# adithom/KWS

Measured on AMD Instinct MI355X. Metric: utterances/sec fwd+bwd, T=99 feat=32 hidden=128, bs=4096 at 1/2/4/8 GPUs, higher is better.
Workload: dtype f32 (split-precision MFMA: exact 3xbf16 planes, fp16 two-plane forward state product; fp32 accumulate)

## Files before the change

include/fastgrnn_hip.h:

```cpp
#ifndef FASTGRNN_HIP_H
#define FASTGRNN_HIP_H

#include <stddef.h>
#include <stdint.h>

#ifdef __cplusplus
extern "C" {
#endif

#define FASTGRNN_HIP_ABI_VERSION 1

typedef enum fastgrnn_status {
  FASTGRNN_OK = 0,
  FASTGRNN_ERR_NULL_POINTER = 1,
  FASTGRNN_ERR_BAD_SHAPE = 2,
  FASTGRNN_ERR_BAD_NONLINEARITY = 3,
  FASTGRNN_ERR_BAD_DTYPE = 4,
  FASTGRNN_ERR_WORKSPACE = 5,
  FASTGRNN_ERR_LAUNCH = 6,
  FASTGRNN_ERR_UNSUPPORTED = 7
} fastgrnn_status;

typedef enum fastgrnn_dtype {
  FASTGRNN_F32 = 0,
  FASTGRNN_F64 = 1,
  FASTGRNN_BF16_IO = 2
} fastgrnn_dtype;

typedef enum fastgrnn_nonlinearity {
  FASTGRNN_NL_SIGMOID = 0, FASTGRNN_NL_RELU = 1, FASTGRNN_NL_TANH = 2,
  FASTGRNN_NL_QUANT_TANH = 3, FASTGRNN_NL_QUANT_SIGM = 4, FASTGRNN_NL_QUANT_SIGM4 = 5
} fastgrnn_nonlinearity;

#define FASTGRNN_FLAG_FORCE_GENERIC 1u
#define FASTGRNN_FLAG_FORCE_F32_MFMA 2u
#define FASTGRNN_FLAG_SAVE_PREACT 4u
#define FASTGRNN_FLAG_FWD_4WAVE 8u
#define FASTGRNN_FLAG_BATCH_MAJOR 16u
#define FASTGRNN_FLAG_X_BFT 128u
#define FASTGRNN_FLAG_FWD_BF16X3 64u
#define FASTGRNN_FLAG_GRAD_LAST 256u
#define FASTGRNN_FLAG_HS_LAST 512u
#define FASTGRNN_FLAG_PREACT_AFFINE 1024u
#define FASTGRNN_FLAG_BN_TRAIN 2048u
#define FASTGRNN_FLAG_ZERO_EXTEND 4096u
#define FASTGRNN_FLAG_NO_INPUT_GRAD 8192u

typedef struct fastgrnn_desc {
  int32_t T, B, F, H;
  int32_t w_rank, u_rank;
  int32_t gate_nl;
  int32_t update_nl;
  int32_t dtype;
  uint32_t flags;
} fastgrnn_desc;

typedef struct fastgrnn_params {
  const void *w, *u;
  const void *w1, *w2, *u1, *u2;
  const void *bias_gate;
  const void *bias_update;
  const void *zeta, *nu;
} fastgrnn_params;

typedef struct fastgrnn_grads {
  void *d_x;
  void *d_bias_gate;
  void *d_bias_update;
  void *d_zeta;
  void *d_nu;
  void *d_h0;
  void *d_w, *d_u;
  void *d_w1, *d_w2;
  void *d_u1, *d_u2;
} fastgrnn_grads;

int fastgrnn_hip_abi_version(void);
const char *fastgrnn_hip_status_string(int status);

int fastgrnn_hip_kernel_path(const fastgrnn_desc *d, int direction);

typedef struct fastgrnn_zext_plan {
  int32_t forward, backward;
  int32_t Hp, Fp;
  int32_t dx_optional, reserved;
  size_t saved_bytes;
} fastgrnn_zext_plan;
int fastgrnn_hip_zero_extend_plan(const fastgrnn_desc *d, fastgrnn_zext_plan *out);

typedef struct fastgrnn_plan {
  int32_t path[2];
  int32_t forward_ws_optional, dx_optional;
  int32_t rank_space_cols, reserved;
  size_t workspace_bytes[2];
  fastgrnn_zext_plan zext;
} fastgrnn_plan;
int fastgrnn_hip_plan(const fastgrnn_desc *d, fastgrnn_plan *out);

size_t fastgrnn_hip_forward_workspace_bytes(const fastgrnn_desc *d);
size_t fastgrnn_hip_backward_workspace_bytes(const fastgrnn_desc *d);

int fastgrnn_hip_forward_unroll(const fastgrnn_desc *d, const fastgrnn_params *p,
                                const void *x, const void *h0,
                                void *hs, void *z_s, void *c_s,
                                void *workspace, size_t workspace_bytes, void *stream);

int fastgrnn_hip_forward_unroll_affine(const fastgrnn_desc *d, const fastgrnn_params *p,
                                       const void *gate_scale, const void *update_scale,
                                       const void *x, const void *h0, void *hs,
                                       void *workspace, size_t workspace_bytes, void *stream);

int fastgrnn_hip_backward_unroll(const fastgrnn_desc *d, const fastgrnn_params *p,
                                 const void *grad_hs, const void *x, const void *hs,
                                 const void *z_s, const void *c_s, const void *h0,
                                 const fastgrnn_grads *g,
                                 void *workspace, size_t workspace_bytes, void *stream);

int fastgrnn_hip_forward(const fastgrnn_desc *d, const fastgrnn_params *p,
                         const void *x, const void *old_h,
                         void *new_h, void *z, void *c,
                         void *workspace, size_t workspace_bytes, void *stream);

int fastgrnn_hip_backward(const fastgrnn_desc *d, const fastgrnn_params *p,
                          const void *grad_h, const void *x, const void *old_h,
                          const void *z, const void *c,
                          const fastgrnn_grads *g,
                          void *workspace, size_t workspace_bytes, void *stream);

size_t fastgrnn_hip_head_workspace_bytes(int32_t B, int32_t H, int32_t C);
// ... 44 lines not shown
```

kws_amd/_lib.py:

```python
from __future__ import annotations

import ctypes as C
import os

_HERE = os.path.dirname(os.path.abspath(__file__))
LIB_PATH = os.environ.get("FASTGRNN_HIP_LIB") or os.path.join(_HERE, "csrc", "libfastgrnn_hip.so")

ABI_VERSION = 1

F32, F64, BF16_IO = 0, 1, 2
FLAG_FORCE_GENERIC = 1
FLAG_FORCE_F32_MFMA = 2
FLAG_SAVE_PREACT = 4
FLAG_FWD_4WAVE = 8
FLAG_FWD_BF16X3 = 64
FLAG_X_BFT = 128
FLAG_GRAD_LAST = 256
FLAG_HS_LAST = 512
FLAG_BATCH_MAJOR = 16
FLAG_PREACT_AFFINE = 1024
FLAG_BN_TRAIN = 2048
FLAG_ZERO_EXTEND = 4096
FLAG_NO_INPUT_GRAD = 8192

NONLINEARITY = {"sigmoid": 0, "relu": 1, "tanh": 2, "quantTanh": 3, "quantSigm": 4, "quantSigm4": 5}

EXPORTS = (
    "fastgrnn_hip_abi_version", "fastgrnn_hip_status_string", "fastgrnn_hip_kernel_path",
    "fastgrnn_hip_forward_workspace_bytes", "fastgrnn_hip_backward_workspace_bytes",
    "fastgrnn_hip_forward_unroll", "fastgrnn_hip_backward_unroll",
    "fastgrnn_hip_forward", "fastgrnn_hip_backward",
    "fastgrnn_hip_head_workspace_bytes", "fastgrnn_hip_head_xent", "fastgrnn_hip_debug_poison_cu_state",
    "fastgrnn_hip_frame_gemm", "fastgrnn_hip_forward_unroll_affine",
    "fastgrnn_hip_bn_train_supported", "fastgrnn_hip_bn_train_forward_workspace_bytes",
    "fastgrnn_hip_bn_train_backward_workspace_bytes", "fastgrnn_hip_bn_train_forward", "fastgrnn_hip_bn_train_backward",
    "fastgrnn_hip_zero_extend_plan", "fastgrnn_hip_plan",
)


class Desc(C.Structure):
    _fields_ = [("T", C.c_int32), ("B", C.c_int32), ("F", C.c_int32), ("H", C.c_int32),
                ("w_rank", C.c_int32), ("u_rank", C.c_int32),
                ("gate_nl", C.c_int32), ("update_nl", C.c_int32),
                ("dtype", C.c_int32), ("flags", C.c_uint32)]


class Params(C.Structure):
    _fields_ = [(n, C.c_void_p) for n in
                ("w", "u", "w1", "w2", "u1", "u2", "bias_gate", "bias_update", "zeta", "nu")]


class Grads(C.Structure):
    _fields_ = [(n, C.c_void_p) for n in
                ("d_x", "d_bias_gate", "d_bias_update", "d_zeta", "d_nu", "d_h0",
                 "d_w", "d_u", "d_w1", "d_w2", "d_u1", "d_u2")]


class BnLayer(C.Structure):
    _fields_ = [("gamma", C.c_void_p), ("beta", C.c_void_p), ("running_mean", C.c_void_p),
                ("running_var", C.c_void_p), ("num_batches_tracked", C.c_void_p),
                ("eps", C.c_double), ("momentum", C.c_double)]


class BnParams(C.Structure):
    _fields_ = [("w", BnLayer), ("u", BnLayer), ("gate", BnLayer), ("update", BnLayer)]


class BnGrads(C.Structure):
    _fields_ = [(n, C.c_void_p) for n in
                ("d_gamma_w", "d_beta_w", "d_gamma_u", "d_beta_u", "d_gamma_gate", "d_beta_gate",
                 "d_gamma_update", "d_beta_update")]


class ZextPlan(C.Structure):
    _fields_ = [("forward", C.c_int32), ("backward", C.c_int32), ("Hp", C.c_int32), ("Fp", C.c_int32),
                ("dx_optional", C.c_int32), ("reserved", C.c_int32), ("saved_bytes", C.c_size_t)]


class Plan(C.Structure):
    _fields_ = [("path", C.c_int32 * 2), ("forward_ws_optional", C.c_int32), ("dx_optional", C.c_int32),
                ("rank_space_cols", C.c_int32), ("reserved", C.c_int32), ("workspace_bytes", C.c_size_t * 2),
                ("zext", ZextPlan)]


class FastGRNNLibraryError(RuntimeError):
    pass


_lib = None


def load():
    global _lib
    if _lib is not None:
        return _lib
    if not os.path.exists(LIB_PATH):
        raise FastGRNNLibraryError(
            "libfastgrnn_hip.so not found at %s -- build it first: "
            "python -c 'import __graft_entry__ as g; g.build()'  (or make -C kws_amd/csrc). "
            "kws_amd has no CPU or eager fallback." % LIB_PATH)
    lib = C.CDLL(LIB_PATH)
    for name in EXPORTS:
        if not hasattr(lib, name):
            raise FastGRNNLibraryError("%s does not export %s" % (LIB_PATH, name))
    vp, sz, i32 = C.c_void_p, C.c_size_t, C.c_int
    DP, PP, GP = C.POINTER(Desc), C.POINTER(Params), C.POINTER(Grads)
# ... 55 lines not shown
```

kws_amd/csrc/kernels_split.hip:

```cpp
#include "split_common.h"

namespace fastgrnn {
namespace {

template <int GATE, int AUX, bool RAGGED>
__global__ __launch_bounds__(256) ONE_WAVE_PER_SIMD void fwd_scan_split(
    int Tn, int B, int rsT, int rsB, const float* __restrict__ x, const float* __restrict__ h0,
    const float* __restrict__ w, const float* __restrict__ u,
    const float* __restrict__ bz, const float* __restrict__ bh,
    const float* __restrict__ zeta, const float* __restrict__ nu,
    float* __restrict__ hs, float* __restrict__ zs, float* __restrict__ cs) {
  constexpr int H = 128, F = 32, MT = 2, KS = H / 32;
  __shared__ u32x4 hl[2][3][KS * 4 * 16];

  const int tid = threadIdx.x;
  const int wv = __builtin_amdgcn_readfirstlane(tid >> 6);
  const int l = tid & 63, i = l & 15, g = l >> 4;
  const int b = blockIdx.x * 16 + i;
  const bool valid = !RAGGED || b < B;
  const int bc = valid ? b : B - 1;
  const int n0 = wv * 32 + g * 8;
  const int myfrag = (wv * 4 + g) * 16 + i;

  Frag3 Uf[MT][KS], Wf[MT];
// ... 68 lines not shown
#pragma unroll
      for (int r = 0; r < 4; ++r) {
        const float pre = a[r];
        const float z = gate_act<GATE>(pre + bzv[mt][r]);
        const float c = ftanh(pre + bhv[mt][r]);
        hown[mt][r] = (sz * (1.0f - z) + sn) * c + hown[mt][r] * z;
        gout.z[mt][r] = (AUX == 2) ? pre : z; gout.c[mt][r] = c;
      }
    };
    constexpr int NM = (KS + 1) * 6;
    SPLIT_STAMP(0)
    if (!FIRST) store_step(t - 1, gprev);
    const f32x4 acc0 = tile_chain(0);
    if (!FIRST) {
      constexpr int NST = (AUX == 1 ? 3 : AUX == 2 ? 2 : 1) * MT, PER = NM / (NST + 1);
#pragma unroll
      for (int j = 0; j < NST; ++j) {
        __builtin_amdgcn_sched_group_barrier(0x008, PER, 0);
        __builtin_amdgcn_sched_group_barrier(0x040, 1, 0);
      }
    }
    __builtin_amdgcn_sched_barrier(0);
    SPLIT_STAMP(1)
    const f32x4 acc1 = tile_chain(1);
    tile_epilogue(0, acc0);
#pragma unroll
    for (int k = 0; k < NM; ++k) {
      __builtin_amdgcn_sched_group_barrier(0x008, 1, 0);
      __builtin_amdgcn_sched_group_barrier(0x002, 3, 0);
    }
    __builtin_amdgcn_sched_barrier(0);
    SPLIT_STAMP(2)
    {
      float probe = acc1[0];
      keep_alive(probe, xB);
#pragma unroll
      for (int s = 0; s < KS; ++s) keep_alive(probe, hB[s]);
      completion_read(probe);
      __builtin_amdgcn_sched_barrier(0);
    }
    tile_epilogue(1, acc1);
    const Frag3 f = split3(hown[0], hown[1]);
#pragma unroll
    for (int p = 0; p < 3; ++p) hl[cur ^ 1][p][myfrag] = f.p[p];
    __builtin_amdgcn_sched_barrier(0);
    SPLIT_STAMP(3)
    lds_barrier();
    SPLIT_STAMP(4)
  };

  Feat xa, xb;
  Gates ga, gb;
  load_x(0, xa);
  __syncthreads();
  step(std::true_type{}, 0, 0, xa, xb, gb, ga);
  int t = 1;
  for (; t + 1 < Tn; t += 2) {
    step(std::false_type{}, t, 1, xb, xa, ga, gb);
    step(std::false_type{}, t + 1, 0, xa, xb, gb, ga);
  }
  if (t < Tn) {
    step(std::false_type{}, t, 1, xb, xa, ga, gb);
    store_step(Tn - 1, gb);
  } else {
    store_step(Tn - 1, ga);
  }
  {
    float probe = hown[0][0];
#pragma unroll
    for (int mt = 0; mt < MT; ++mt) {
      keep_alive(probe, Wf[mt]);
#pragma unroll
      for (int s = 0; s < KS; ++s) keep_alive(probe, Uf[mt][s]);
    }
  }
#ifdef FASTGRNN_DIAG_STAMPS
  if (blockIdx.x == 7 && l == 0) { for (int k = 0; k < 8; ++k) g_sdiag[wv][k] = dsum[k]; }
#endif
}

constexpr int W8_ROWH = 272;
constexpr int W8_ROWX = 80;

constexpr bool fwd_w8_built(int gate, int aux, bool bf, bool f16h, bool prein, bool uq, bool aff) {
  const bool ref_gate = gate <= FASTGRNN_NL_TANH;
  if (f16h && !gate_bounds_state(gate)) return false;
  if (aff) return ref_gate && !bf && !uq && (aux == 0 || aux == 3);
  if (uq) return !bf && !prein && (aux == 0 || aux == 2);
  if (bf && prein) return ref_gate && (aux == 0 || aux == 2);
  return true;
}
template <int GATE, int AUX, bool RAGGED, bool BF = false, bool F16H = true, bool PREIN = false, bool UQ = false,
          bool AFF = false>
__global__ __launch_bounds__(512) void fwd_scan_split_w8(
    int Tn, int B, int rsT, int rsB, int mode, const float* __restrict__ x, const float* __restrict__ h0,
    const float* __restrict__ w, const float* __restrict__ u,
    const float* __restrict__ bz, const float* __restrict__ bh,
    const float* __restrict__ zeta, const float* __restrict__ nu,
    float* __restrict__ hs, float* __restrict__ zs, float* __restrict__ cs,
    const float* __restrict__ sg = nullptr, const float* __restrict__ sc = nullptr) {
  constexpr int H = 128, F = 32, KS = H / 32;
  __shared__ __attribute__((aligned(16))) unsigned char hpl[2][3][16 * W8_ROWH];
  __shared__ __attribute__((aligned(16))) unsigned char xpl[PREIN ? 1 : 2][3][PREIN ? 16 : 16 * W8_ROWX];
  float* const pbuf = (AUX == 1) ? cs : zs;

  const int tid = threadIdx.x;
  const int wv = __builtin_amdgcn_readfirstlane(tid >> 6);
  const int l = tid & 63, i = l & 15, g = l >> 4;
  const int b = blockIdx.x * 16 + i;
  const bool valid = !RAGGED || b < B;
  const int bc = valid ? b : B - 1;
  const int n0 = wv * 16 + g * 4;
  const bool xbft = (mode & 1) != 0;
  constexpr bool hs_last = AUX == 3;
  const int xu = tid >> 5, xf = tid & 31;
  const int xb = blockIdx.x * 16 + xu;
  const int xbc = (!RAGGED || xb < B) ? xb : B - 1;

  const f32x4 bzv = ld4(bz + n0), bhv = ld4(bh + n0);
  const f32x4 sgv = AFF ? ld4(sg + n0) : f32x4{1.f, 1.f, 1.f, 1.f}, scv = AFF ? ld4(sc + n0) : f32x4{1.f, 1.f, 1.f, 1.f};
  f32x4 hown = ld4(h0 + (size_t)bc * H + n0);
  const float sz = fsigmoid(zeta[0]), sn = fsigmoid(nu[0]);

  bool use_h16 = false;
  if constexpr (F16H) {
    __shared__ float hmax_s[8];
    float hm = fmaxf(fmaxf(fabsf(hown[0]), fabsf(hown[1])), fmaxf(fabsf(hown[2]), fabsf(hown[3])));
    if (!(hm == hm)) hm = 3.0e38f;
#pragma unroll
    for (int m = 1; m < 64; m <<= 1) hm = fmaxf(hm, __shfl_xor(hm, m));
    if (l == 0) hmax_s[wv] = hm;
    __syncthreads();
#pragma unroll
    for (int k2 = 0; k2 < 8; ++k2) hm = fmaxf(hm, hmax_s[k2]);
    use_h16 = __builtin_amdgcn_readfirstlane((int)(hm + (float)Tn + 2.0f < 3.0e4f)) != 0;
  }

  auto scan = [&](auto h16_tag) __attribute__((always_inline)) {
  constexpr bool H16 = decltype(h16_tag)::value;
  Frag3 Uf[KS], Wf;
  Frag2h Uh[KS];
  float u_unscale = 1.0f;
  {
    const int nA = wv * 16 + i;
    f32x4 ulo[KS], uhi[KS];
    float umax = 0.f;
#pragma unroll
    for (int s2 = 0; s2 < KS; ++s2) {
      const float* up = u + (size_t)nA * H + 32 * s2 + 8 * g;
      ulo[s2] = ld4(up); uhi[s2] = ld4(up + 4);
#pragma unroll
      for (int j = 0; j < 4; ++j) umax = fmaxf(umax, fmaxf(fabsf(ulo[s2][j]), fabsf(uhi[s2][j])));
    }
    if (H16) {
#pragma unroll
      for (int m = 1; m < 64; m <<= 1) umax = fmaxf(umax, __shfl_xor(umax, m));
      int e = 0;
      if (umax > 0.f && umax < 3.0e38f) (void)frexpf(umax, &e);
      e = e < -100 ? -100 : (e > 100 ? 100 : e);
      const float u_scale = ldexpf(1.0f, 13 - e);
      u_unscale = ldexpf(1.0f, e - 13);
#pragma unroll
      for (int s2 = 0; s2 < KS; ++s2) Uh[s2] = split2h8(ulo[s2] * u_scale, uhi[s2] * u_scale);
    } else {
#pragma unroll
      for (int s2 = 0; s2 < KS; ++s2) Uf[s2] = split3(ulo[s2], uhi[s2]);
    }
    if (!PREIN) {
      const float* wp = w + (size_t)nA * F + 8 * g;
      Wf = split3(ld4(wp), ld4(wp + 4));
    }
  }

  auto publish_h = [&](int buf) __attribute__((always_inline)) {
    const unsigned off = i * W8_ROWH + n0 * 2;
    if (H16) {
      uint2 hi, lo;
      split2h(hown[0], hown[1], hi.x, lo.x); split2h(hown[2], hown[3], hi.y, lo.y);
      *reinterpret_cast<uint2*>(&hpl[buf][0][off]) = hi;
      *reinterpret_cast<uint2*>(&hpl[buf][1][off]) = lo;
      return;
    }
    uint2 q0, q1, q2;
    split_quad(hown, q0, q1, q2);
    *reinterpret_cast<uint2*>(&hpl[buf][0][off]) = q0;
    *reinterpret_cast<uint2*>(&hpl[buf][1][off]) = q1;
    *reinterpret_cast<uint2*>(&hpl[buf][2][off]) = q2;
  };
  auto publish_x = [&](int buf, float v) __attribute__((always_inline)) {
    unsigned short s0, s1, s2;
    split_one(v, s0, s1, s2);
    const unsigned off = xu * W8_ROWX + xf * 2;
    *reinterpret_cast<unsigned short*>(&xpl[buf][0][off]) = s0;
    *reinterpret_cast<unsigned short*>(&xpl[buf][1][off]) = s1;
    *reinterpret_cast<unsigned short*>(&xpl[buf][2][off]) = s2;
  };
  const size_t xbase = xbft ? ((size_t)xbc * F + xf) * Tn : (size_t)xbc * rsB * F + xf;
  const size_t xstep = xbft ? 1 : (size_t)rsT * F;
  auto load_x = [&](int t) __attribute__((always_inline)) {
    const size_t e = xbase + (size_t)t * xstep;
    return BF ? bf16_to_f32(reinterpret_cast<const unsigned short*>(x)[e]) : x[e];
  };
  auto load_p = [&](int t) __attribute__((always_inline)) {
    return ld4(pbuf + ((size_t)t * rsT + (size_t)bc * rsB) * H + n0);
  };
  auto store_step = [&](int t, const f32x4 aux) __attribute__((always_inline)) {
    if (hs_last && t != Tn - 1) return;
    if (RAGGED) lds_writes_landed();
    if (valid) {
      const size_t o = hs_last ? (size_t)b * H + n0 : ((size_t)t * rsT + (size_t)b * rsB) * H + n0;
      if (BF) st4_bf16(reinterpret_cast<unsigned short*>(hs) + o, hown); else st4(hs + o, hown);
      if (AUX == 2) st4(zs + o, aux);
    }
  };

  publish_h(0);
  float xnext = 0.f;
  f32x4 pnext = f32x4{0.f, 0.f, 0.f, 0.f};
  if (PREIN) {
    pnext = load_p(0);
  } else {
    publish_x(0, load_x(0));
    xnext = load_x(Tn > 1 ? 1 : 0);
  }
  __syncthreads();

  f32x4 aux_prev = f32x4{0.f, 0.f, 0.f, 0.f};
#ifdef FASTGRNN_DIAG_STAMPS
  unsigned long long dsum[8] = {0, 0, 0, 0, 0, 0, 0, 0}, dlast = 0;
  asm volatile("s_memtime %0\n\ts_waitcnt lgkmcnt(0)" : "=s"(dlast)::"memory");
#endif
  for (int t = 0; t < Tn; ++t) {
    const int cur = t & 1;
    SPLIT_STAMP(0)
    const float xpub = xnext;
    const f32x4 pcur = pnext;
    if (PREIN) pnext = load_p(t + 1 < Tn ? t + 1 : Tn - 1);
    else xnext = load_x(t + 2 < Tn ? t + 2 : Tn - 1);
    Frag3 xB, hB[KS];
    Frag2h hH[KS];
    if (!PREIN) {
#pragma unroll
      for (int p = 0; p < 3; ++p) xB.p[p] = *reinterpret_cast<const u32x4*>(&xpl[cur][p][i * W8_ROWX + 16 * g]);
    }
#pragma unroll
    for (int s2 = 0; s2 < KS; ++s2) {
      if (H16) {
        hH[s2].hi = *reinterpret_cast<const u32x4*>(&hpl[cur][0][i * W8_ROWH + 64 * s2 + 16 * g]);
        hH[s2].lo = *reinterpret_cast<const u32x4*>(&hpl[cur][1][i * W8_ROWH + 64 * s2 + 16 * g]);
      } else {
#pragma unroll
        for (int p = 0; p < 3; ++p)
          hB[s2].p[p] = *reinterpret_cast<const u32x4*>(&hpl[cur][p][i * W8_ROWH + 64 * s2 + 16 * g]);
      }
    }
    if (t > 0) store_step(t - 1, aux_prev);
    if (!PREIN) publish_x(cur ^ 1, xpub);
    __builtin_amdgcn_sched_barrier(0);
    SPLIT_STAMP(1)
    f32x4 a = f32x4{0.f, 0.f, 0.f, 0.f}, alo = a;
    if (PREIN) {
      a = pcur;
    } else if (BF) {
      alo = mfma_bf16(Wf.p[2], xB.p[0], alo);
      alo = mfma_bf16(Wf.p[1], xB.p[0], alo);
      a = mfma_bf16(Wf.p[0], xB.p[0], a);
    } else {
      mfma6_hl(Wf, xB, a, alo);
    }
    if (H16) {
      f32x4 ah = f32x4{0.f, 0.f, 0.f, 0.f}, ahlo = ah;
#pragma unroll
      for (int s2 = 0; s2 < KS; ++s2) mfma3h_hl(Uh[s2], hH[s2], ah, ahlo);
      a = (a + alo) + (ah + ahlo) * u_unscale;
    } else {
#pragma unroll
      for (int s2 = 0; s2 < KS; ++s2) mfma6_hl(Uf[s2], hB[s2], a, alo);
      a += alo;
    }
    f32x4 zq, cq;
    SPLIT_STAMP(2)
#pragma unroll
    for (int r = 0; r < 4; ++r) {
      const float z = gate_act<GATE>(AFF ? fmaf(a[r], sgv[r], bzv[r]) : a[r] + bzv[r]);
      const float c = UQ ? fminf(fmaxf(a[r] + bhv[r], -1.0f), 1.0f)
                         : ftanh(AFF ? fmaf(a[r], scv[r], bhv[r]) : a[r] + bhv[r]);
      hown[r] = (sz * (1.0f - z) + sn) * c + hown[r] * z;
      zq[r] = z; cq[r] = c;
    }
    if (AUX == 1 && RAGGED) lds_writes_landed();
    if (AUX == 1 && valid) {
      const size_t o = ((size_t)t * rsT + (size_t)b * rsB) * H + n0;
      st4(zs + o, zq); st4(cs + o, cq);
    }
    aux_prev = a;
    publish_h(cur ^ 1);
    SPLIT_STAMP(3)
    lds_barrier();
    SPLIT_STAMP(4)
  }
#ifdef FASTGRNN_DIAG_STAMPS
  if (blockIdx.x == 7 && l == 0) { for (int k2 = 0; k2 < 8; ++k2) g_sdiag[wv][k2] = dsum[k2]; }
#endif
  store_step(Tn - 1, aux_prev);
  };
  if constexpr (F16H) {
    if (use_h16) scan(std::true_type{}); else scan(std::false_type{});
  } else {
    scan(std::false_type{});
  }
}



constexpr int SLAB = (128 * 128 + 128 * 32 + 2 * 128 + 2 + 63) & ~63;

constexpr int ROW_H = 288;
constexpr int ROW_X = 96;
constexpr int PLANE_H = 16 * ROW_H;
constexpr int PLANE_X = 16 * ROW_X;
constexpr int IMG = 2 * 3 * PLANE_H + 3 * PLANE_X;

constexpr int OFF_DP = 0, OFF_HP = 3 * PLANE_H, OFF_XP = 6 * PLANE_H;

template <bool WITH_DX>
struct BwdW8Lds {
  unsigned char img[4][IMG];
  f32x4 DX[2][8][64];
  float bias[2][128];
  float red[16];
};
template <>
struct BwdW8Lds<false> {
  unsigned char img[4][IMG];
  float bias[2][128];
  float red[16];
};

constexpr bool bwd_w8_built(int gate, bool preact, bool bf, bool nox, bool uq, bool nodx) {
  const bool ref_gate = gate <= FASTGRNN_NL_TANH;
  if (nox) return !uq && !nodx && (!bf || (ref_gate && preact));
  if (uq) return preact && !bf;
  if (bf) return preact;
  return true;
}
template <int GATE, bool PREACT, bool RAGGED, bool BF = false, bool NOX = false, bool UQ = false, bool NODX = false>
__global__ __launch_bounds__(512) void bwd_scan_split_w8(
    int Tn, int B, int rsT, int rsB, int mode, const float* __restrict__ ghs, const float* __restrict__ x,
    const float* __restrict__ hs, const float* __restrict__ aux0, const float* __restrict__ aux1,
    const float* __restrict__ h0, const float* __restrict__ w, const float* __restrict__ u,
    const float* __restrict__ bz, const float* __restrict__ bh,
    const float* __restrict__ zeta, const float* __restrict__ nu,
    float* __restrict__ d_x, float* __restrict__ d_h0, float* __restrict__ part) {
  constexpr int H = 128, F = 32, KS = 4, NFT = NOX ? 0 : 2, NC = NOX ? 4 : 5;
  static_assert(!(NOX && NODX), "NOX scans leave d_x to a GEMM of its own");
  __shared__ BwdW8Lds<!NODX> S;
#ifdef FASTGRNN_DIAG_STAMPS
  unsigned long long dsum[8] = {0, 0, 0, 0, 0, 0, 0, 0}, dlast = 0;
  asm volatile("s_memtime %0\n\ts_waitcnt lgkmcnt(0)" : "=s"(dlast)::"memory");
#endif

  const bool xbft = (mode & 1) != 0, g_last = (mode & 2) != 0;
  const int tid = threadIdx.x;
  const int wv = __builtin_amdgcn_readfirstlane(tid >> 6);
  const int l = tid & 63, i = l & 15, g = l >> 4;
  const int b = blockIdx.x * 16 + i;
  const bool valid = !RAGGED || b < B;
  const int bc = valid ? b : B - 1;
  const int n0 = wv * 16 + g * 4;
  const float sz = fsigmoid(zeta[0]), sn = fsigmoid(nu[0]);
  if (Tn & 1) {
    for (int idx = tid; idx < IMG / 4; idx += 512) reinterpret_cast<unsigned*>(&S.img[Tn & 3][0])[idx] = 0u;
  }
  if (PREACT && tid < 256) S.bias[tid >> 7][tid & 127] = (tid < 128 ? bz : bh)[tid & 127];

  Frag3 UTf[KS];
#pragma unroll
  for (int s2 = 0; s2 < KS; ++s2) {
    f32x4 lo, hi;
#pragma unroll
    for (int j = 0; j < 4; ++j) {
      lo[j] = u[(size_t)(32 * s2 + 8 * g + j) * H + wv * 16 + i];
      hi[j] = u[(size_t)(32 * s2 + 8 * g + 4 + j) * H + wv * 16 + i];
    }
    UTf[s2] = split3(lo, hi);
  }
  const int xf2 = wv & 1, xks = wv >> 1;
// ... 361 lines not shown
#pragma unroll
    for (int j = 0; j < 16; ++j) t += sm[j][o];
    const int oW = H * H, oBz = oW + H * F, oBh = oBz + H, oZ = oBh + H;
    if (idx < oW) d_u[idx] = t;
    else if (idx < oBz) { if (d_w) d_w[idx - oW] = t; }
    else if (idx < oBh) d_bz[idx - oBz] = t;
    else if (idx < oZ) d_bh[idx - oBh] = t;
    else if (idx == oZ) { const float sz = 1.0f / (1.0f + expf(-zeta[0])); d_zeta[0] = t * sz * (1.0f - sz); }
    else { const float sn = 1.0f / (1.0f + expf(-nu[0])); d_nu[0] = t * sn * (1.0f - sn); }
  }
}

bool dense_wide_shape(const fastgrnn_desc& d) {
  return d.w_rank == 0 && d.u_rank == 0 && d.H == 128 && (d.F == 64 || d.F == 128 || d.F == 256) &&
         ((double)d.T * d.B + 16.0) * (d.F > 128 ? d.F : 128) * 4.0 < 4294967296.0;
}
struct WideBwdWs { size_t slabs, dpre, tn, xtm, total; };
WideBwdWs wide_bwd_layout(const fastgrnn_desc& d) {
  const size_t TB = (size_t)d.T * d.B, nwg = (d.B + 15) / 16;
  WideBwdWs L; size_t o = 0;
  L.slabs = o; o += align256(nwg * SLAB * 4);
  L.dpre = o; o += align256((TB + 16) * 128 * 4);
  L.tn = o; o += tn_gemm_big_ws(TB, 128, d.F);
  L.xtm = o; if (d.flags & FASTGRNN_FLAG_X_BFT) o += align256(TB * (size_t)d.F * 4);
  L.total = o;
  return L;
}

struct BwdW8 { int gate; bool preact, ragged, bf, nox, uq, nodx; };

bool launch_bwd_w8(const fastgrnn_desc& d, const fastgrnn_params& p, const void* ghs, const void* x, const void* hs,
                   const void* a0, const void* a1, const void* h0, const fastgrnn_grads& g, void* ws, hipStream_t s) {
  const int nwg = (d.B + 15) / 16;
  dim3 grid(nwg);
  const bool wide = dense_wide_shape(d);
  const WideBwdWs L = wide ? wide_bwd_layout(d) : WideBwdWs{0, 0, 0, 0, 0};
  float* part = reinterpret_cast<float*>(ws);
  float* dpre = wide ? reinterpret_cast<float*>(reinterpret_cast<char*>(ws) + L.dpre) : nullptr;
  auto go8 = [&](auto kern) __attribute__((always_inline)) {
    hipLaunchKernelGGL(kern, grid, dim3(512), 0, s, d.T, d.B, row_stride_t(d), row_stride_b(d),
                       ((d.flags & FASTGRNN_FLAG_X_BFT) ? 1 : 0) | ((d.flags & FASTGRNN_FLAG_GRAD_LAST) ? 2 : 0), (const float*)ghs,
                       (const float*)x, (const float*)hs,
                       (const float*)a0, (const float*)a1, (const float*)h0, (const float*)p.w, (const float*)p.u,
                       (const float*)p.bias_gate, (const float*)p.bias_update, (const float*)p.zeta,
                       (const float*)p.nu, wide ? dpre : (float*)g.d_x, (float*)g.d_h0, part);
  };
  const BwdW8 v{d.gate_nl, (d.flags & FASTGRNN_FLAG_SAVE_PREACT) != 0, (d.B % 16) != 0, d.dtype == FASTGRNN_BF16_IO,
                wide, d.update_nl == FASTGRNN_NL_QUANT_TANH, !wide && g.d_x == nullptr};
  const bool launched =
      pick_int<0, 1, 2, 3, 4, 5>(v.gate, [&](auto G_) {
      return pick_bool(v.preact, [&](auto PA_) {
      return pick_bool(v.bf, [&](auto BF_) {
      return pick_bool(v.nox, [&](auto NX_) {
      return pick_bool(v.uq, [&](auto UQ_) {
      return pick_bool(v.nodx, [&](auto ND_) {
      return pick_bool(v.ragged, [&](auto RG_) {
        constexpr int G = decltype(G_)::value;
        constexpr bool PA = decltype(PA_)::value, BF = decltype(BF_)::value, NX = decltype(NX_)::value,
                       UQ = decltype(UQ_)::value, ND = decltype(ND_)::value, RG = decltype(RG_)::value;
        if constexpr (bwd_w8_built(G, PA, BF, NX, UQ, ND)) { go8(bwd_scan_split_w8<G, PA, RG, BF, NX, UQ, ND>); return true; }
        else return false;
      }); }); }); }); }); }); });
  if (!launched) return false;
  const int ntot = 128 * 128 + 128 * 32 + 2 * 128 + 2;
  hipLaunchKernelGGL(reduce_slabs_split, dim3((ntot + 63) / 64), dim3(1024), 0, s, nwg, part, (const float*)p.zeta,
                     (const float*)p.nu, (float*)g.d_u, wide ? (float*)nullptr : (float*)g.d_w, (float*)g.d_bias_gate,
                     (float*)g.d_bias_update, (float*)g.d_zeta, (float*)g.d_nu);
  if (wide) {
    const size_t TB = (size_t)d.T * d.B;
    const bool bfw = d.dtype == FASTGRNN_BF16_IO;
    const bool bft = (d.flags & FASTGRNN_FLAG_X_BFT) != 0;
    float* xtm = reinterpret_cast<float*>(reinterpret_cast<char*>(ws) + L.xtm);
    if (bft) { bft_transpose_f32(d.B, d.T, (const float*)x, xtm, true, s, d.F); x = xtm; }
    tn_gemm_big_run(TB, 128, d.F, dpre, 128, (const float*)x, x, (size_t)0, d.F,
                    reinterpret_cast<float*>(reinterpret_cast<char*>(ws) + L.tn), (float*)g.d_w, d.F, s, bfw);
    if (g.d_x) {
      rows_gemm(TB, d.F, 128, true, dpre, (const float*)p.w, bft ? (void*)xtm : g.d_x, false, bfw, s);
      if (bft) bft_transpose_f32(d.B, d.T, xtm, (float*)g.d_x, false, s, d.F);
    }
  }
  return true;
}

struct FwdW8 { int gate, aux; bool ragged, bf, f16h, prein, uq, aff; };

bool launch_fwd(const fastgrnn_desc& d, const fastgrnn_params& p, const void* x, const void* h0, void* hs,
                void* zs, void* cs, hipStream_t s, void* pws, const float* sg, const float* sc) {
  dim3 grid((d.B + 15) / 16), block(256);
  const bool ragged = (d.B % 16) != 0, bf = d.dtype == FASTGRNN_BF16_IO, prein = pws != nullptr;
  const int aux = zs == nullptr ? 0 : ((d.flags & FASTGRNN_FLAG_SAVE_PREACT) ? 2 : 1);
  if (prein && aux == 0) zs = pws;
  auto go = [&](auto kern) __attribute__((always_inline)) {
    hipLaunchKernelGGL(kern, grid, block, 0, s, d.T, d.B, row_stride_t(d), row_stride_b(d), (const float*)x,
                       (const float*)h0, (const float*)p.w,
                       (const float*)p.u, (const float*)p.bias_gate, (const float*)p.bias_update,
                       (const float*)p.zeta, (const float*)p.nu, (float*)hs, (float*)zs, (float*)cs);
  };
  auto go8 = [&](auto kern) __attribute__((always_inline)) {
    hipLaunchKernelGGL(kern, grid, dim3(512), 0, s, d.T, d.B, row_stride_t(d), row_stride_b(d),
                       (d.flags & FASTGRNN_FLAG_X_BFT) ? 1 : 0, (const float*)x, (const float*)h0, (const float*)p.w,
                       (const float*)p.u, (const float*)p.bias_gate, (const float*)p.bias_update,
                       (const float*)p.zeta, (const float*)p.nu, (float*)hs, (float*)zs, (float*)cs, sg, sc);
  };
  if ((d.flags & FASTGRNN_FLAG_FWD_4WAVE) && !sg && !bf && d.gate_nl <= FASTGRNN_NL_TANH &&
      !(d.flags & (FASTGRNN_FLAG_X_BFT | FASTGRNN_FLAG_HS_LAST | FASTGRNN_FLAG_FWD_BF16X3)))
    return pick_int<0, 1, 2>(d.gate_nl, [&](auto G_) {
           return pick_int<0, 1, 2>(aux, [&](auto A_) {
           return pick_bool(ragged, [&](auto RG_) {
             go(fwd_scan_split<decltype(G_)::value, decltype(A_)::value, decltype(RG_)::value>);
             return true;
           }); }); });
  const FwdW8 v{d.gate_nl, (d.flags & FASTGRNN_FLAG_HS_LAST) ? 3 : aux, ragged, bf,
                gate_bounds_state(d.gate_nl) && !(d.flags & FASTGRNN_FLAG_FWD_BF16X3), prein,
                d.update_nl == FASTGRNN_NL_QUANT_TANH, sg != nullptr};
  return pick_int<0, 1, 2, 3, 4, 5>(v.gate, [&](auto G_) {
         return pick_int<0, 1, 2, 3>(v.aux, [&](auto A_) {
         return pick_bool(v.bf, [&](auto BF_) {
         return pick_bool(v.f16h, [&](auto FH_) {
         return pick_bool(v.prein, [&](auto PI_) {
         return pick_bool(v.uq, [&](auto UQ_) {
         return pick_bool(v.aff, [&](auto AF_) {
         return pick_bool(v.ragged, [&](auto RG_) {
           constexpr int G = decltype(G_)::value, A = decltype(A_)::value;
           constexpr bool BF = decltype(BF_)::value, FH = decltype(FH_)::value, PI = decltype(PI_)::value,
                          UQ = decltype(UQ_)::value, AF = decltype(AF_)::value, RG = decltype(RG_)::value;
           if constexpr (fwd_w8_built(G, A, BF, FH, PI, UQ, AF)) { go8(fwd_scan_split_w8<G, A, RG, BF, FH, PI, UQ, AF>); return true; }
           else return false;
         }); }); }); }); }); }); }); });
}

}

bool split_supported(const fastgrnn_desc& d, int direction) {
  if ((d.dtype != FASTGRNN_F32 && d.dtype != FASTGRNN_BF16_IO) ||
      (d.update_nl != FASTGRNN_NL_TANH && d.update_nl != FASTGRNN_NL_QUANT_TANH) ||
      d.gate_nl < FASTGRNN_NL_SIGMOID || d.gate_nl > FASTGRNN_NL_QUANT_SIGM4)
    return false;
  if (d.update_nl == FASTGRNN_NL_QUANT_TANH) {
    const bool shape = d.w_rank == 0 && d.u_rank == 0 && d.H == 128 && d.F == 32 && d.dtype == FASTGRNN_F32 && seq_fits32(d);
    if (!shape || (d.flags & (FASTGRNN_FLAG_X_BFT | FASTGRNN_FLAG_HS_LAST | FASTGRNN_FLAG_FWD_4WAVE))) return false;
    return direction == 0 || (d.flags & FASTGRNN_FLAG_SAVE_PREACT) != 0;
  }
  const bool dense = d.w_rank == 0 && d.u_rank == 0 && d.H == 128 && d.F == 32 && seq_fits32(d);
  const bool preact = (d.flags & FASTGRNN_FLAG_SAVE_PREACT) != 0;
  if (h256_shape(d)) return h256_supported(d, direction);
  if (lowrank_shape(d)) return lowrank_supported(d, direction);
  if (densified_shape(d)) return densified_supported(d, direction);
  if (dense_wide_shape(d)) {
    if ((d.flags & FASTGRNN_FLAG_X_BFT) &&
        (d.dtype != FASTGRNN_F32 || (direction == 1 && (d.flags & FASTGRNN_FLAG_BATCH_MAJOR)))) return false;
    if (d.dtype == FASTGRNN_BF16_IO)
      return d.gate_nl <= FASTGRNN_NL_TANH &&
             !(d.flags & (FASTGRNN_FLAG_HS_LAST | FASTGRNN_FLAG_GRAD_LAST)) && (direction == 0 || preact);
    if (direction == 0 && preact && (d.flags & FASTGRNN_FLAG_HS_LAST)) return false;
    return d.gate_nl <= FASTGRNN_NL_TANH || direction == 0 || preact;
  }
  if (d.gate_nl > FASTGRNN_NL_TANH || (d.flags & FASTGRNN_FLAG_X_BFT)) return dense && (direction == 0 || preact);
  if (d.flags & (FASTGRNN_FLAG_GRAD_LAST | FASTGRNN_FLAG_HS_LAST)) {
    if (!dense) return false;
    if (direction == 0 && (d.flags & FASTGRNN_FLAG_SAVE_PREACT) && (d.flags & FASTGRNN_FLAG_HS_LAST)) return false;
  }
  if (d.dtype == FASTGRNN_BF16_IO) return dense && (direction == 0 || preact);
  return dense;
}

bool affine_supported(const fastgrnn_desc& d) {
  if (d.dtype != FASTGRNN_F32 || d.gate_nl > FASTGRNN_NL_TANH || d.update_nl != FASTGRNN_NL_TANH) return false;
  if (d.flags & (FASTGRNN_FLAG_SAVE_PREACT | FASTGRNN_FLAG_GRAD_LAST)) return false;
  if ((d.flags & FASTGRNN_FLAG_X_BFT) && !((h256_shape(d) && d.F != 32) || dense_wide_shape(d))) return false;
  if (h256_shape(d)) return h256_supported(d, 0);
  return (d.w_rank == 0 && d.u_rank == 0 && d.H == 128 && d.F == 32 && seq_fits32(d)) || dense_wide_shape(d);
}

size_t split_forward_ws(const fastgrnn_desc& d) {
  if (dense_wide_shape(d)) return align256((size_t)d.T * d.B * 128 * 4);
  if (h256_shape(d)) return h256_forward_ws(d);
  if (lowrank_shape(d)) return lowrank_forward_ws(d);
  if (densified_shape(d)) return densified_forward_ws(d);
  return 0;
}

bool split_forward_ws_optional(const fastgrnn_desc& d) { return dense_wide_shape(d); }
bool split_dx_optional(const fastgrnn_desc& d) { return dense_wide_shape(d) || h256_shape(d); }
bool split_dx_skippable(const fastgrnn_desc& d) { return d.w_rank == 0 && d.u_rank == 0 && d.H == 128 && d.F == 32; }

size_t split_backward_ws(const fastgrnn_desc& d) {
  if (h256_shape(d)) return h256_backward_ws(d);
  if (dense_wide_shape(d)) return wide_bwd_layout(d).total;
  if (lowrank_shape(d)) return lowrank_backward_ws(d);
  if (densified_shape(d)) return densified_backward_ws(d);
  return align256((size_t)((d.B + 15) / 16) * SLAB * 4);
}

int split_backward(const fastgrnn_desc& d, const fastgrnn_params& p, const void* ghs, const void* x, const void* hs,
                   const void* zs, const void* cs, const void* h0, const fastgrnn_grads& g, void* ws,
                   hipStream_t s) {
  if (h256_shape(d)) return h256_backward(d, p, ghs, x, hs, zs, cs, h0, g, ws, s);
  if (lowrank_shape(d)) return lowrank_backward(d, p, ghs, x, hs, zs, cs, h0, g, ws, s);
  if (densified_shape(d)) return densified_backward(d, p, ghs, x, hs, zs, cs, h0, g, ws, s);
  if (!launch_bwd_w8(d, p, ghs, x, hs, zs, cs, h0, g, ws, s)) return FASTGRNN_ERR_UNSUPPORTED;
  return hipGetLastError() == hipSuccess ? FASTGRNN_OK : FASTGRNN_ERR_LAUNCH;
}

int split_forward(const fastgrnn_desc& d, const fastgrnn_params& p, const void* x, const void* h0, void* hs,
                  void* zs, void* cs, void* ws, hipStream_t s, const void* sg_, const void* sc_) {
  if (!(d.flags & FASTGRNN_FLAG_SAVE_PREACT) && (zs == nullptr) != (cs == nullptr)) return FASTGRNN_ERR_NULL_POINTER;
  if (d.dtype == FASTGRNN_BF16_IO && zs && !(d.flags & FASTGRNN_FLAG_SAVE_PREACT)) return FASTGRNN_ERR_UNSUPPORTED;
  const float* sg = reinterpret_cast<const float*>(sg_);
  const float* sc = reinterpret_cast<const float*>(sc_);
  if (sg && (zs || !affine_supported(d))) return FASTGRNN_ERR_UNSUPPORTED;
  if (h256_shape(d)) return h256_forward(d, p, x, h0, hs, zs, cs, ws, s, sg, sc);
// ... 17 lines not shown
```

kws_amd/csrc/split_common.h:

```cpp
#pragma once
#include "common.h"
#include "variant_pick.h"
#include <type_traits>
#include <utility>

namespace fastgrnn {
namespace {

typedef float f32x4 __attribute__((ext_vector_type(4)));
typedef __bf16 bf16x8 __attribute__((ext_vector_type(8)));
typedef unsigned int u32x4 __attribute__((ext_vector_type(4)));
typedef short s16x4 __attribute__((ext_vector_type(4)));
typedef short s16x8 __attribute__((ext_vector_type(8)));
typedef __attribute__((address_space(3))) s16x4 lds_s16x4;

constexpr float LOG2E = 1.4426950408889634f;

__device__ __forceinline__ float fsigmoid(float a) {
  return __builtin_amdgcn_rcpf(1.0f + __builtin_amdgcn_exp2f(-LOG2E * a));
}
__device__ __forceinline__ float ftanh(float a) {
  return 1.0f - 2.0f * __builtin_amdgcn_rcpf(1.0f + __builtin_amdgcn_exp2f((2.0f * LOG2E) * a));
}
template <int GATE> __device__ __forceinline__ float gate_act(float a) {
// ... 111 lines not shown
  const _Float16 ha = (_Float16)a, hb = (_Float16)b;
  const _Float16 la = (_Float16)(a - (float)ha), lb = (_Float16)(b - (float)hb);
  hi = __builtin_bit_cast(unsigned, f16x2{ha, hb});
  lo = __builtin_bit_cast(unsigned, f16x2{la, lb});
}
__device__ __forceinline__ void split3h(float a, float b, unsigned& p0, unsigned& p1, unsigned& p2) {
  const _Float16 ha = (_Float16)a, hb = (_Float16)b;
  const float ra = a - (float)ha, rb = b - (float)hb;
  const _Float16 la = (_Float16)ra, lb = (_Float16)rb;
  const _Float16 ma = (_Float16)(ra - (float)la), mb = (_Float16)(rb - (float)lb);
  p0 = __builtin_bit_cast(unsigned, f16x2{ha, hb});
  p1 = __builtin_bit_cast(unsigned, f16x2{la, lb});
  p2 = __builtin_bit_cast(unsigned, f16x2{ma, mb});
}
__device__ __forceinline__ Frag2h split2h8(const f32x4 lo4, const f32x4 hi4) {
  unsigned h[4], l[4];
  split2h(lo4[0], lo4[1], h[0], l[0]); split2h(lo4[2], lo4[3], h[1], l[1]);
  split2h(hi4[0], hi4[1], h[2], l[2]); split2h(hi4[2], hi4[3], h[3], l[3]);
  Frag2h f;
  f.hi = u32x4{h[0], h[1], h[2], h[3]}; f.lo = u32x4{l[0], l[1], l[2], l[3]};
  return f;
}
__device__ __forceinline__ f32x4 mfma_f16(u32x4 a, u32x4 b, f32x4 c) {
  return __builtin_amdgcn_mfma_f32_16x16x32_f16(__builtin_bit_cast(f16x8, a), __builtin_bit_cast(f16x8, b), c, 0, 0, 0);
}
__device__ __forceinline__ f32x4 mfma3h(const Frag2h& a, const Frag2h& b, f32x4 acc) {
  acc = mfma_f16(a.lo, b.hi, acc);
  acc = mfma_f16(a.hi, b.lo, acc);
  acc = mfma_f16(a.hi, b.hi, acc);
  return acc;
}

__device__ __forceinline__ void mfma3h_hl(const Frag2h& a, const Frag2h& b, f32x4& hi, f32x4& lo) {
  lo = mfma_f16(a.lo, b.hi, lo);
  lo = mfma_f16(a.hi, b.lo, lo);
  hi = mfma_f16(a.hi, b.hi, hi);
}

__device__ __forceinline__ f32x4 mfma6(const Frag3& a, const Frag3& b, f32x4 acc) {
  acc = mfma_bf16(a.p[2], b.p[0], acc);
  acc = mfma_bf16(a.p[1], b.p[1], acc);
  acc = mfma_bf16(a.p[0], b.p[2], acc);
  acc = mfma_bf16(a.p[1], b.p[0], acc);
  acc = mfma_bf16(a.p[0], b.p[1], acc);
  acc = mfma_bf16(a.p[0], b.p[0], acc);
  return acc;
}

__device__ __forceinline__ void mfma6_hl(const Frag3& a, const Frag3& b, f32x4& hi, f32x4& lo) {
  lo = mfma_bf16(a.p[2], b.p[0], lo);
  lo = mfma_bf16(a.p[1], b.p[1], lo);
  lo = mfma_bf16(a.p[0], b.p[2], lo);
  lo = mfma_bf16(a.p[1], b.p[0], lo);
  lo = mfma_bf16(a.p[0], b.p[1], lo);
  hi = mfma_bf16(a.p[0], b.p[0], hi);
}

struct Half3 { s16x4 p[3]; };
__device__ __forceinline__ f32x4 mfma_bf16_k16(s16x4 a, s16x4 b, f32x4 c) {
  return __builtin_amdgcn_mfma_f32_16x16x16bf16_1k(a, b, c, 0, 0, 0);
}
__device__ __forceinline__ f32x4 mfma6_k16(const Half3& a, const Half3& b, f32x4 acc) {
  acc = mfma_bf16_k16(a.p[2], b.p[0], acc);
  acc = mfma_bf16_k16(a.p[1], b.p[1], acc);
  acc = mfma_bf16_k16(a.p[0], b.p[2], acc);
  acc = mfma_bf16_k16(a.p[1], b.p[0], acc);
  acc = mfma_bf16_k16(a.p[0], b.p[1], acc);
  acc = mfma_bf16_k16(a.p[0], b.p[0], acc);
  return acc;
}

__device__ __forceinline__ void mfma6_hl_k16(const Half3& a, const Half3& b, f32x4& hi, f32x4& lo) {
  lo = mfma_bf16_k16(a.p[2], b.p[0], lo);
  lo = mfma_bf16_k16(a.p[1], b.p[1], lo);
  lo = mfma_bf16_k16(a.p[0], b.p[2], lo);
  lo = mfma_bf16_k16(a.p[1], b.p[0], lo);
  lo = mfma_bf16_k16(a.p[0], b.p[1], lo);
  hi = mfma_bf16_k16(a.p[0], b.p[0], hi);
}

__device__ __forceinline__ void keep_alive(float& tie, const Frag3& f) {
  asm volatile("" : "+v"(tie) : "v"(f.p[0]), "v"(f.p[1]), "v"(f.p[2]));
}

template <typename Fn, int... Is>
__device__ __forceinline__ void static_for_impl(Fn&& f, std::integer_sequence<int, Is...>) {
  (f(std::integral_constant<int, Is>{}), ...);
}
template <int N, typename Fn>
__device__ __forceinline__ void static_for(Fn&& f) { static_for_impl(f, std::make_integer_sequence<int, N>{}); }


__device__ __forceinline__ u32x4 tr_frag(unsigned lds_byte_addr, int rowb) {
  const s16x4 lo = __builtin_amdgcn_ds_read_tr16_b64_v4i16(reinterpret_cast<lds_s16x4*>((size_t)lds_byte_addr));
  const s16x4 hi = __builtin_amdgcn_ds_read_tr16_b64_v4i16(reinterpret_cast<lds_s16x4*>((size_t)(lds_byte_addr + 4 * rowb)));
  const s16x8 v = __builtin_shufflevector(lo, hi, 0, 1, 2, 3, 4, 5, 6, 7);
  return __builtin_bit_cast(u32x4, v);
}

static inline int row_stride_t(const fastgrnn_desc& d) { return (d.flags & FASTGRNN_FLAG_BATCH_MAJOR) ? 1 : d.B; }
static inline int row_stride_b(const fastgrnn_desc& d) { return (d.flags & FASTGRNN_FLAG_BATCH_MAJOR) ? d.T : 1; }
static inline bool seq_fits32(const fastgrnn_desc& d) {
  return (double)d.T * d.B * (d.H > d.F ? d.H : d.F) * 4.0 < 4294967296.0;
}

}
}
```

Measured before the change: 11.37 million.

## Stagger forward scan wave roles so half the waves prefetch next step's products

```diff
diff --git a/include/fastgrnn_hip.h b/include/fastgrnn_hip.h
--- a/include/fastgrnn_hip.h
+++ b/include/fastgrnn_hip.h
@@ -45,6 +45,7 @@
 #define FASTGRNN_FLAG_BN_TRAIN 2048u
 #define FASTGRNN_FLAG_ZERO_EXTEND 4096u
 #define FASTGRNN_FLAG_NO_INPUT_GRAD 8192u
+#define FASTGRNN_FLAG_FWD_LOCKSTEP 16384u
 
 typedef struct fastgrnn_desc {
   int32_t T, B, F, H;
diff --git a/kws_amd/_lib.py b/kws_amd/_lib.py
--- a/kws_amd/_lib.py
+++ b/kws_amd/_lib.py
@@ -22,6 +22,7 @@
 FLAG_BN_TRAIN = 2048
 FLAG_ZERO_EXTEND = 4096
 FLAG_NO_INPUT_GRAD = 8192
+FLAG_FWD_LOCKSTEP = 16384
 
 NONLINEARITY = {"sigmoid": 0, "relu": 1, "tanh": 2, "quantTanh": 3, "quantSigm": 4, "quantSigm4": 5}
 
diff --git a/kws_amd/csrc/kernels_split.hip b/kws_amd/csrc/kernels_split.hip
--- a/kws_amd/csrc/kernels_split.hip
+++ b/kws_amd/csrc/kernels_split.hip
@@ -174,8 +174,12 @@
 constexpr int W8_ROWH = 272;
 constexpr int W8_ROWX = 80;
 
-constexpr bool fwd_w8_built(int gate, int aux, bool bf, bool f16h, bool prein, bool uq, bool aff) {
+constexpr bool fwd_w8_staggers(int aux, bool bf, bool prein, bool uq, bool aff) {
+  return !bf && !prein && !uq && !aff && aux != 1;
+}
+constexpr bool fwd_w8_built(int gate, int aux, bool bf, bool f16h, bool prein, bool uq, bool aff, bool stag) {
   const bool ref_gate = gate <= FASTGRNN_NL_TANH;
+  if (stag && !fwd_w8_staggers(aux, bf, prein, uq, aff)) return false;
   if (f16h && !gate_bounds_state(gate)) return false;
   if (aff) return ref_gate && !bf && !uq && (aux == 0 || aux == 3);
   if (uq) return !bf && !prein && (aux == 0 || aux == 2);
@@ -183,7 +187,7 @@
   return true;
 }
 template <int GATE, int AUX, bool RAGGED, bool BF = false, bool F16H = true, bool PREIN = false, bool UQ = false,
-          bool AFF = false>
+          bool AFF = false, bool STAG = false>
 __global__ __launch_bounds__(512) void fwd_scan_split_w8(
     int Tn, int B, int rsT, int rsB, int mode, const float* __restrict__ x, const float* __restrict__ h0,
     const float* __restrict__ w, const float* __restrict__ u,
@@ -306,6 +310,17 @@
     }
   };
 
+  auto cell = [&](const f32x4 a, f32x4& zq, f32x4& cq) __attribute__((always_inline)) {
+#pragma unroll
+    for (int r = 0; r < 4; ++r) {
+      const float z = gate_act<GATE>(AFF ? fmaf(a[r], sgv[r], bzv[r]) : a[r] + bzv[r]);
+      const float c = UQ ? fminf(fmaxf(a[r] + bhv[r], -1.0f), 1.0f)
+                         : ftanh(AFF ? fmaf(a[r], scv[r], bhv[r]) : a[r] + bhv[r]);
+      hown[r] = (sz * (1.0f - z) + sn) * c + hown[r] * z;
+      zq[r] = z; cq[r] = c;
+    }
+  };
+
   publish_h(0);
   float xnext = 0.f;
   f32x4 pnext = f32x4{0.f, 0.f, 0.f, 0.f};
@@ -322,6 +337,102 @@
   unsigned long long dsum[8] = {0, 0, 0, 0, 0, 0, 0, 0}, dlast = 0;
   asm volatile("s_memtime %0\n\ts_waitcnt lgkmcnt(0)" : "=s"(dlast)::"memory");
 #endif
+  if constexpr (STAG) {
+  auto role = [&](auto role_tag) __attribute__((always_inline)) {
+    constexpr bool EARLY = decltype(role_tag)::value;
+    const f32x4 z4 = f32x4{0.f, 0.f, 0.f, 0.f};
+    f32x4 a = z4, alo = z4, ah = z4, ahlo = z4;
+    Frag3 xB, hB[KS];
+    Frag2h hH[KS];
+    auto read_x = [&](int buf) __attribute__((always_inline)) {
+#pragma unroll
+      for (int p = 0; p < 3; ++p) xB.p[p] = *reinterpret_cast<const u32x4*>(&xpl[buf][p][i * W8_ROWX + 16 * g]);
+    };
+    auto read_h = [&](int buf, auto s_tag) __attribute__((always_inline)) {
+      constexpr int s2 = decltype(s_tag)::value;
+      if (H16) {
+        hH[s2].hi = *reinterpret_cast<const u32x4*>(&hpl[buf][0][i * W8_ROWH + 64 * s2 + 16 * g]);
+        hH[s2].lo = *reinterpret_cast<const u32x4*>(&hpl[buf][1][i * W8_ROWH + 64 * s2 + 16 * g]);
+      } else {
+#pragma unroll
+        for (int p = 0; p < 3; ++p)
+          hB[s2].p[p] = *reinterpret_cast<const u32x4*>(&hpl[buf][p][i * W8_ROWH + 64 * s2 + 16 * g]);
+      }
+    };
+    auto frame_product = [&]() __attribute__((always_inline)) {
+      a = z4; alo = z4; ah = z4; ahlo = z4;
+      mfma6_hl(Wf, xB, a, alo);
+    };
+    auto state_product = [&](auto s_tag) __attribute__((always_inline)) {
+      constexpr int s2 = decltype(s_tag)::value;
+      if (H16) mfma3h_hl(Uh[s2], hH[s2], ah, ahlo); else mfma6_hl(Uf[s2], hB[s2], a, alo);
+    };
+    auto next_frame = [&](int t, int cur) __attribute__((always_inline)) {
+      const float xpub = xnext;
+      xnext = load_x(t + 2 < Tn ? t + 2 : Tn - 1);
+      publish_x(cur ^ 1, xpub);
+    };
+    auto finish = [&](int cur) __attribute__((always_inline)) {
+      if (H16) a = (a + alo) + (ah + ahlo) * u_unscale; else a += alo;
+      f32x4 zq, cq;
+      cell(a, zq, cq);
+      aux_prev = a;
+      publish_h(cur ^ 1);
+    };
+    using K0 = std::integral_constant<int, 0>; using K1 = std::integral_constant<int, 1>;
+    using K2 = std::integral_constant<int, 2>; using K3 = std::integral_constant<int, 3>;
+    auto early_odd = [&](auto first_tag, int t, int nxt) __attribute__((always_inline)) {
+      read_x(nxt); read_h(nxt, K0{}); read_h(nxt, K1{});
+      if constexpr (!decltype(first_tag)::value && !hs_last) store_step(t, aux_prev);
+      __builtin_amdgcn_sched_barrier(0);
+      SPLIT_STAMP(5)
+      frame_product(); state_product(K0{}); state_product(K1{});
+      __builtin_amdgcn_sched_barrier(0);
+      completion_read(H16 ? (a[0] + alo[0]) + (ah[0] + ahlo[0]) : a[0] + alo[0]);
+      __builtin_amdgcn_sched_barrier(0);
+      SPLIT_STAMP(6)
+    };
+    if constexpr (EARLY) early_odd(std::true_type{}, -1, 0);
+    for (int t = 0; t < Tn; ++t) {
+      const int cur = t & 1;
+      SPLIT_STAMP(0)
+      if constexpr (EARLY) {
+        read_h(cur, K2{}); read_h(cur, K3{});
+        next_frame(t, cur);
+        __builtin_amdgcn_sched_barrier(0);
+        SPLIT_STAMP(1)
+        state_product(K2{}); state_product(K3{});
+        SPLIT_STAMP(2)
+        finish(cur);
+        SPLIT_STAMP(3)
+      } else {
+        read_x(cur); read_h(cur, K0{}); read_h(cur, K1{}); read_h(cur, K2{}); read_h(cur, K3{});
+        if constexpr (!hs_last) { if (t > 0) store_step(t - 1, aux_prev); }
+        next_frame(t, cur);
+        __builtin_amdgcn_sched_barrier(0);
+        SPLIT_STAMP(1)
+        frame_product(); state_product(K0{}); state_product(K1{}); state_product(K2{}); state_product(K3{});
+        __builtin_amdgcn_sched_barrier(0);
+        SPLIT_STAMP(2)
+      }
+      lds_barrier();
+      SPLIT_STAMP(4)
+      if constexpr (EARLY) {
+        early_odd(std::false_type{}, t, cur ^ 1);
+      } else {
+        finish(cur);
+        SPLIT_STAMP(3)
+      }
+      lds_barrier();
+      SPLIT_STAMP(7)
+    }
+#ifdef FASTGRNN_DIAG_STAMPS
+    if (blockIdx.x == 7 && l == 0) { for (int k2 = 0; k2 < 8; ++k2) g_sdiag[wv][k2] = dsum[k2]; }
+#endif
+    if (!EARLY || hs_last) store_step(Tn - 1, aux_prev);
+  };
+  if (wv < 4) role(std::true_type{}); else role(std::false_type{});
+  } else {
   for (int t = 0; t < Tn; ++t) {
     const int cur = t & 1;
     SPLIT_STAMP(0)
@@ -372,14 +483,7 @@
     }
     f32x4 zq, cq;
     SPLIT_STAMP(2)
-#pragma unroll
-    for (int r = 0; r < 4; ++r) {
-      const float z = gate_act<GATE>(AFF ? fmaf(a[r], sgv[r], bzv[r]) : a[r] + bzv[r]);
-      const float c = UQ ? fminf(fmaxf(a[r] + bhv[r], -1.0f), 1.0f)
-                         : ftanh(AFF ? fmaf(a[r], scv[r], bhv[r]) : a[r] + bhv[r]);
-      hown[r] = (sz * (1.0f - z) + sn) * c + hown[r] * z;
-      zq[r] = z; cq[r] = c;
-    }
+    cell(a, zq, cq);
     if (AUX == 1 && RAGGED) lds_writes_landed();
     if (AUX == 1 && valid) {
       const size_t o = ((size_t)t * rsT + (size_t)b * rsB) * H + n0;
@@ -395,6 +499,7 @@
   if (blockIdx.x == 7 && l == 0) { for (int k2 = 0; k2 < 8; ++k2) g_sdiag[wv][k2] = dsum[k2]; }
 #endif
   store_step(Tn - 1, aux_prev);
+  }
   };
   if constexpr (F16H) {
     if (use_h16) scan(std::true_type{}); else scan(std::false_type{});
@@ -922,7 +1027,7 @@
   return true;
 }
 
-struct FwdW8 { int gate, aux; bool ragged, bf, f16h, prein, uq, aff; };
+struct FwdW8 { int gate, aux; bool ragged, bf, f16h, prein, uq, aff, stag; };
 
 bool launch_fwd(const fastgrnn_desc& d, const fastgrnn_params& p, const void* x, const void* h0, void* hs,
                 void* zs, void* cs, hipStream_t s, void* pws, const float* sg, const float* sc) {
@@ -950,9 +1055,11 @@
              go(fwd_scan_split<decltype(G_)::value, decltype(A_)::value, decltype(RG_)::value>);
              return true;
            }); }); });
-  const FwdW8 v{d.gate_nl, (d.flags & FASTGRNN_FLAG_HS_LAST) ? 3 : aux, ragged, bf,
-                gate_bounds_state(d.gate_nl) && !(d.flags & FASTGRNN_FLAG_FWD_BF16X3), prein,
-                d.update_nl == FASTGRNN_NL_QUANT_TANH, sg != nullptr};
+  const int aux8 = (d.flags & FASTGRNN_FLAG_HS_LAST) ? 3 : aux;
+  const bool uq = d.update_nl == FASTGRNN_NL_QUANT_TANH, aff = sg != nullptr;
+  const FwdW8 v{d.gate_nl, aux8, ragged, bf,
+                gate_bounds_state(d.gate_nl) && !(d.flags & FASTGRNN_FLAG_FWD_BF16X3), prein, uq, aff,
+                fwd_w8_staggers(aux8, bf, prein, uq, aff) && !(d.flags & FASTGRNN_FLAG_FWD_LOCKSTEP)};
   return pick_int<0, 1, 2, 3, 4, 5>(v.gate, [&](auto G_) {
          return pick_int<0, 1, 2, 3>(v.aux, [&](auto A_) {
          return pick_bool(v.bf, [&](auto BF_) {
@@ -960,13 +1067,15 @@
          return pick_bool(v.prein, [&](auto PI_) {
          return pick_bool(v.uq, [&](auto UQ_) {
          return pick_bool(v.aff, [&](auto AF_) {
+         return pick_bool(v.stag, [&](auto SG_) {
          return pick_bool(v.ragged, [&](auto RG_) {
            constexpr int G = decltype(G_)::value, A = decltype(A_)::value;
            constexpr bool BF = decltype(BF_)::value, FH = decltype(FH_)::value, PI = decltype(PI_)::value,
-                          UQ = decltype(UQ_)::value, AF = decltype(AF_)::value, RG = decltype(RG_)::value;
-           if constexpr (fwd_w8_built(G, A, BF, FH, PI, UQ, AF)) { go8(fwd_scan_split_w8<G, A, RG, BF, FH, PI, UQ, AF>); return true; }
+                          UQ = decltype(UQ_)::value, AF = decltype(AF_)::value, SG = decltype(SG_)::value,
+                          RG = decltype(RG_)::value;
+           if constexpr (fwd_w8_built(G, A, BF, FH, PI, UQ, AF, SG)) { go8(fwd_scan_split_w8<G, A, RG, BF, FH, PI, UQ, AF, SG>); return true; }
            else return false;
-         }); }); }); }); }); }); }); });
+         }); }); }); }); }); }); }); }); });
 }
 
 }
diff --git a/kws_amd/csrc/split_common.h b/kws_amd/csrc/split_common.h
--- a/kws_amd/csrc/split_common.h
+++ b/kws_amd/csrc/split_common.h
@@ -217,6 +217,9 @@
 __device__ __forceinline__ void keep_alive(float& tie, const Frag3& f) {
   asm volatile("" : "+v"(tie) : "v"(f.p[0]), "v"(f.p[1]), "v"(f.p[2]));
 }
+__device__ __forceinline__ void keep_alive(float& tie, const Frag2h& f) {
+  asm volatile("" : "+v"(tie) : "v"(f.hi), "v"(f.lo));
+}
 
 template <typename Fn, int... Is>
 __device__ __forceinline__ void static_for_impl(Fn&& f, std::integer_sequence<int, Is...>) {
```

Result: no change. 11.40 million (median of 5 runs) (+0.3%).
